# Ipsedo/MARLClassification

Hardware: AMD Instinct MI355X
Metric: agent-env-steps/sec (higher is better)
Workload: dtype f32; 1 GPU; RESISC45 256x256x3, 16 agents, 16 steps, f=12, README dims (configs[2]); full train iteration: rollout + A2C loss + BPTT backward + Adam; batch_per_gpu=256, global_batch=256, parallelism=dp1, rng=library (Philox4x32-10), launch=eager

## Files before the change

### marlclassification_amd/csrc/cnn.hip

```cpp
#include <stdlib.h>

#include <type_traits>

#include "common.h"

namespace marl {

template <bool FROM_OBS, typename PIX>
__global__ __launch_bounds__(256) void gather_im2col_kernel(
    const PIX* __restrict__ img, const int32_t* __restrict__ pos, float* __restrict__ cols,
    int ldk, int64_t rows, int nb, int c_img, int cin, int H, int W, int f, int rb) {
    extern __shared__ __attribute__((aligned(16))) float patch[];
    const int ff = f * f;
    const int pe = cin * ff;
    const int64_t row0 = (int64_t)blockIdx.x * rb;
    int nrow = (int)(rows - row0 < rb ? rows - row0 : rb);
    for (int idx = threadIdx.x; idx < nrow * pe; idx += 256) {
        const int lr = idx / pe, e = idx % pe;
        const int ci = e / ff, y = (e % ff) / f, x = e % f;
        const int64_t r = row0 + lr;
        float v;
        if (FROM_OBS) {
            v = (float)img[((r * c_img + ci) * f + y) * f + x];
        } else {
// ... 36 lines not shown
    const int rb = gather_rb(cin, f);
    const size_t lds = (size_t)rb * cin * f * f * sizeof(float);
    if (lds > 64 * 1024) {
        set_error("window %d too large for the gather kernel", f);
        return MARL_ELIMIT;
    }
    if (img_u8)
        hipLaunchKernelGGL((gather_im2col_kernel<false, unsigned char>),
                           dim3((unsigned)cdiv(rows, rb)), dim3(256), lds, st,
                           static_cast<const unsigned char*>(img), pos, cols, ldk, rows, nb, c_img,
                           cin, H, W, f, rb);
    else
        hipLaunchKernelGGL((gather_im2col_kernel<false, float>), dim3((unsigned)cdiv(rows, rb)),
                           dim3(256), lds, st, static_cast<const float*>(img), pos, cols, ldk, rows,
                           nb, c_img, cin, H, W, f, rb);
    MARL_LAUNCH_CHECK();
    return MARL_OK;
}

int launch_obs_im2col(const float* obs, float* cols, int ldk, int64_t rows, int c_img, int cin,
                      int f, hipStream_t st) {
    const int rb = gather_rb(cin, f);
    const size_t lds = (size_t)rb * cin * f * f * sizeof(float);
    if (lds > 64 * 1024) return MARL_ELIMIT;
    hipLaunchKernelGGL((gather_im2col_kernel<true, float>), dim3((unsigned)cdiv(rows, rb)), dim3(256),
                       lds, st, obs, (const int32_t*)nullptr, cols, ldk, rows, 1, c_img, cin, 0, 0,
                       f, rb);
    MARL_LAUNCH_CHECK();
    return MARL_OK;
}

#ifdef MARL_KERNEL_TS
int ts_begin(long long** dev, int call) {
    if (!*dev) (void)hipMalloc(dev, 16 * 48 * sizeof(long long));
    const char* e = getenv("MARL_TS_CALL");
    const int want = e ? atoi(e) : 100;
    if (call != want) return 0;
    (void)hipMemset(*dev, 0, 16 * 48 * sizeof(long long));
    return 1;
}
void ts_report(const char* tag, long long* dev, int waves) {
    static long long h[16 * 48];
    (void)hipMemcpy(h, dev, sizeof(h), hipMemcpyDeviceToHost);
    for (int w = 0; w < waves; w += (waves > 1 ? waves - 1 : 1)) {
        const long long* t = h + w * 48;
        fprintf(stderr, "[ts] %s wave %d/%d:", tag, w, waves);
        long long tot = 0;
        for (int i = 1; i < 48 && t[i]; ++i) {
            fprintf(stderr, " %lld", t[i] - t[i - 1]);
            tot += t[i] - t[i - 1];
        }
        fprintf(stderr, " | total %.2f us\n", tot / 100.0);
    }
}
#endif

typedef float cf32x4 __attribute__((ext_vector_type(4)));

__device__ __forceinline__ float cnn_silu(float y) { return silu_fast(y); }

__global__ __launch_bounds__(512) void cnn_fwd_kernel(const CnnFwdArgs A) {
    extern __shared__ __attribute__((aligned(16))) float lds[];
    float* patch = lds;
    float* gstat = lds + A.off_stat;
    __shared__ int64_t simg[16];
    __shared__ int spos[16][2];
    const int tid = threadIdx.x, lane = tid & 63, wave = tid >> 6;
    const int nthreads = blockDim.x, nwaves = nthreads >> 6;
    const int quad = lane >> 4, l16 = lane & 15;
    const int64_t row0 = (int64_t)blockIdx.x * A.rb;
    const int nrow = (int)(A.rows - row0 < A.rb ? A.rows - row0 : A.rb);

#ifdef MARL_KERNEL_TS
    MARL_TS_DECL(A.ts);
#endif
    MARL_TS();
    if (tid < nrow) {
        const int64_t r = row0 + tid;
        if (A.obs) {
            simg[tid] = r * A.c_img * A.f * A.f;
            spos[tid][0] = spos[tid][1] = 0;
        } else {
            simg[tid] = (r % A.nb) * A.c_img * (int64_t)A.H * A.W;
            spos[tid][0] = A.pos[r * 2];
            spos[tid][1] = A.pos[r * 2 + 1];
// ... 2876 lines not shown
```

### marlclassification_amd/csrc/common.h

```cpp
#pragma once

#include <hip/hip_runtime.h>
#include <stdint.h>
#include <stdio.h>

#include "../../include/marl_hip.h"
#include "split.h"

namespace marl {

constexpr int kWave = 64;

inline int p4(int x) { return (x + 3) & ~3; }
inline int64_t cdiv(int64_t a, int64_t b) { return (a + b - 1) / b; }

void set_error(const char* fmt, ...);

int tune_get(const char* key, int dflt);
int tune_set(const char* key, int value);

__device__ __forceinline__ float rcp_fast(float x) { return __builtin_amdgcn_rcpf(x); }
__device__ __forceinline__ float sigmoid_acc(float x) { return rcp_fast(1.0f + __expf(-x)); }
__device__ __forceinline__ float tanh_fast(float x) { return 1.0f - 2.0f * rcp_fast(1.0f + __expf(2.0f * x)); }
__device__ __forceinline__ float silu_fast(float y) { return y * sigmoid_acc(y); }
// ... 409 lines not shown

struct PanelLayer {
    const float* w;
    int ldw;
    const float* bias;
    const float* gamma;
    const float* beta;
    int n;
    float* z;
    int ldz;
    float* stats;
    float* a;
    int lda;
    char* a3;
    int a3_row0, a3_steps, a3_col0;
};
constexpr int kPanelMaxLayers = 4;
struct PanelFwdProb {
    const float* x;
    int ldx, k0;
    int agg_na, agg_nb;
    float* xbar;
    int m, nlayers;
    PanelLayer layer[kPanelMaxLayers];
    int by_batch, g_na, g_nb, agg_at, ld_xbar;
    const float* mix;
};
struct PanelFwdBatch {
    PanelFwdProb p[2];
    int count;
    int off_panel1, off_red, off_part, off_prm;
    int off_mix;
    int has_sample, panel_blocks;
    int ln_narrow_max;
    SampleArgs sample;
#ifdef MARL_KERNEL_TS
    long long* ts;
#endif
};
int panel_chain_supported(int na, int n_msg, int threads);
int panel_supported(int k0, int n0, int n1);
int launch_panel_fwd(PanelFwdBatch& b, hipStream_t st);

struct LstmBwdArgs {
    const float* dh;
    float* dc;
    float* gates;
    const float* c_prev;
    const float* c_new;
    int lddh, lddc, ldg, ldc, n;
    char* g3;
    int g3_row0, g3_steps;
    int skip_f32;
};
struct LstmBwdBatch {
    LstmBwdArgs a[2];
    int64_t rows;
    int vec4;
};
inline bool lstm_bwd_vec4_ok(const LstmBwdArgs& a) {
    return (a.n & 3) == 0 && (a.lddh & 3) == 0 && (a.lddc & 3) == 0 && (a.ldg & 3) == 0 && (a.ldc & 3) == 0;
}
__device__ __forceinline__ void lstm_cell_bwd_at(const LstmBwdArgs& A, int64_t r, int u, float dhv);
__device__ __forceinline__ void lstm_cell_bwd_elem(const LstmBwdArgs& A, int64_t rows, int64_t idx) {
    const int n = A.n;
    if (idx >= rows * n) return;
    const int64_t r = idx / n;
    const int u = (int)(idx % n);
    lstm_cell_bwd_at(A, r, u, A.dh[r * A.lddh + u]);
}
__device__ __forceinline__ void lstm_cell_bwd_at(const LstmBwdArgs& A, int64_t r, int u, float dhv) {
    const int n = A.n;
    float* g = A.gates + r * A.ldg + u;
    const float gi = g[0], gf = g[n], gg = g[2 * n], go = g[3 * n];
// ... 69 lines not shown
};
struct PanelBwdProb {
    const float* da;
    int ldda;
    const float* da2;
    int ldda2;
    int agg_na, agg_nb;
    int m, nlayers;
    PanelBwdLayer layer[kPanelMaxLayers];
    float* dx;
    int lddx, accumulate;
    int by_batch, g_na, g_nb, agg_at;
    int has_cellb;
    LstmBwdArgs cellb;
    int off_e, off_prm, off_colp, off_part, off_rowmap;
    const float* mix;
    int off_mix;
    int tail_lds;
    int has_cell, panel_blocks;
    LstmBwdArgs cell;
    int64_t cell_rows;
    int cell_vec4;
    int cellb_img_done, cell_img_done;
#ifdef MARL_KERNEL_TS
    long long* ts;
#endif
};
int panel_bwd_blocks(int m);
int panel_chain_blocks(int na, int nb);
int panel_chain_by_batch(int na);
int launch_panel_bwd(PanelBwdProb& p, hipStream_t st);

#ifdef MARL_KERNEL_TS
#define MARL_TS_DECL(ptr) long long* ts_ = (ptr); int tsi_ = 0
#define MARL_TS()                                                                         \
    if (ts_ && (threadIdx.x & 63) == 0 && blockIdx.x == 37 && blockIdx.y == 0 && tsi_ < 48) \
    ts_[(threadIdx.x >> 6) * 48 + tsi_++] = wall_clock64()
int ts_begin(long long** dev, int call);
void ts_report(const char* tag, long long* dev, int waves);
#else
#define MARL_TS_DECL(ptr)
#define MARL_TS()
#endif

struct FDiv {
    uint32_t d, m;
};
inline FDiv make_fdiv(int d) { return FDiv{(uint32_t)d, (uint32_t)(((1ull << 32) / (uint64_t)d) + 1)}; }
__device__ __forceinline__ int fdiv(int n, FDiv f) {
    return f.d == 1 ? n : (int)__umulhi((uint32_t)n, f.m);
}

struct CnnFwdLayer {
    const float *w, *bias, *gamma, *beta;
    float* cols;
    float* z;
    float* gst;
    int cin, cout, G, hin, hout, P, K, ldk;
    const float* wfrag;
};
struct CnnFwdArgs {
    const void* img;
    const float* obs;
    const int32_t* pos;
    int img_u8;
    int64_t rows;
    int nb, c_img, H, W, f, L;
    CnnFwdLayer layer[MARL_MAX_CNN_LAYERS];
    float* u;
    int ldu;
    char* u3;
    int u3_row0, u3_steps;
// ... 161 lines not shown
```

### marlclassification_amd/csrc/episode.hip

```cpp
#include <math.h>
#include <stdlib.h>
#include <string.h>

#include "common.h"

namespace marl {

struct Dims {
    int na, nb, ns;
    int64_t R, NR;
    int H, W, c_img, f;
    int L;
    int ch[MARL_MAX_CNN_LAYERS + 1];
    int grp[MARL_MAX_CNN_LAYERS];
    int hw[MARL_MAX_CNN_LAYERS + 1];
    int P[MARL_MAX_CNN_LAYERS];
    int K[MARL_MAX_CNN_LAYERS];
    int ldk[MARL_MAX_CNN_LAYERS];
    int nf, nin;
    int n_b, n_a, n_m, nm2, n_mo, n_d, nA, nC, nlb, nla;
    int ld_nin, ld_nb, ld_na, ld_nm, ld_nm2, ld_nmo, ld_nd, ld_nla, ld_nlb, ld_gb, ld_ga, ld_nC,
        ld_nA;
    int ld_dbl;
};
// ... 856 lines not shown
                                 c.at(c.e.ZE1, t), d.ld_nm2, R, d.nm2, c.wp(MARL_P_ENC_B0)),
                       gemm_prob(c.HCs(t + 1), d.ld_na, c.wp(MARL_P_POL_W0), d.ld_na, d.n_a,
                                 c.at(c.e.ZP1, t), d.ld_nla, R, d.nla, c.wp(MARL_P_POL_B0))));
    } else if (which == 1) {
        MARL_TRY(gemm1(c, gemm_prob(c.Hs(t + 1), d.ld_nb, c.wp(MARL_P_ENC_W0), d.ld_nb, d.n_b,
                                    c.at(c.e.ZE1, t), d.ld_nm2, R, d.nm2, c.wp(MARL_P_ENC_B0))));
    } else {
        MARL_TRY(gemm1(c, gemm_prob(c.HCs(t + 1), d.ld_na, c.wp(MARL_P_POL_W0), d.ld_na, d.n_a,
                                    c.at(c.e.ZP1, t), d.ld_nla, R, d.nla, c.wp(MARL_P_POL_B0))));
    }
    if (which & 2)
        MARL_TRY(launch_ln_silu_fwd(c.at(c.e.ZP1, t), d.ld_nla, c.wp(MARL_P_POL_LNW),
                                    c.wp(MARL_P_POL_LNB), c.at(c.e.AP1, t), d.ld_nla,
                                    c.at(c.e.STP1, t), d.R, d.nla, st));
    if (which & 1) {
        MARL_TRY(launch_ln_silu_fwd(c.at(c.e.ZE1, t), d.ld_nm2, c.wp(MARL_P_ENC_LN0W),
                                    c.wp(MARL_P_ENC_LN0B), c.at(c.e.AE1, t), d.ld_nm2,
                                    c.at(c.e.STE1, t), d.R, d.nm2, st));
        MARL_TRY(gemm1(c, gemm_prob(c.at(c.e.AE1, t), d.ld_nm2, c.wp(MARL_P_ENC_W1), d.ld_nm2,
                                    d.nm2, c.at(c.e.ZE2, t), d.ld_nm, R, d.n_m,
                                    c.wp(MARL_P_ENC_B1))));
        MARL_TRY(launch_ln_silu_fwd(c.at(c.e.ZE2, t), d.ld_nm, c.wp(MARL_P_ENC_LN1W),
                                    c.wp(MARL_P_ENC_LN1B), c.MSGs(t + 1), d.ld_nm,
                                    c.at(c.e.STE2, t), d.R, d.n_m, st));
    }
    return MARL_OK;
}

static bool use_chain(const Dims& d) {
    return use_panels(d) && panel_chain_supported(d.na, d.n_m, 256) && d.n_mo <= 384 && d.nm2 <= 384 &&
           d.n_m <= 384 && tune_get("panel_chain", 1) != 0 &&
           (!g_comm || d.n_b <= 384);
}
static int step_chain(const Ctx& c, int t) {
    const Dims& d = c.d;
    PanelFwdBatch pb{};
    pb.count = 2;
    PanelFwdProb& pe = pb.p[0];
    fill_enc_prob(c, t, pe);
    pe.by_batch = panel_chain_by_batch(d.na);
    pe.g_na = d.na;
    pe.g_nb = d.nb;
    if (t + 1 < d.ns) {
        fill_dec_layers(c, t + 1, pe.layer + 2);
        pe.nlayers = 4;
        pe.agg_at = 2;
        pe.xbar = c.at(c.e.MBAR, t + 1);
        pe.ld_xbar = d.ld_nm;
        pe.mix = g_comm;
    }
    fill_pol_prob(c, t, pb.p[1]);
    return launch_panel_fwd(pb, c.st);
}

static int step_core(const Ctx& c, int t, const StepIn& in) {
    MARL_TRY(step_cnn(c, t, in));
    MARL_TRY(step_decode(c, t));
    MARL_TRY(step_pos_lstm(c, t, in));
    return step_encode_policy(c, t, 3);
}

struct SideStream {
    hipStream_t s = nullptr;
    hipEvent_t ev[64];
    int next = 0;
    int init() {
        if (s) return MARL_OK;
        MARL_HIP_CHECK(hipStreamCreateWithFlags(&s, hipStreamNonBlocking));
        for (auto& e : ev) MARL_HIP_CHECK(hipEventCreateWithFlags(&e, hipEventDisableTiming));
        return MARL_OK;
    }
    int order(hipStream_t from, hipStream_t to) {
        hipEvent_t e = ev[next];
        next = (next + 1) % 64;
        MARL_HIP_CHECK(hipEventRecord(e, from));
        MARL_HIP_CHECK(hipStreamWaitEvent(to, e, 0));
        return MARL_OK;
    }
};
static SideStream g_side;

static bool use_side_stream() {
    static int enabled = -1;
    (void)enabled;
// ... 968 lines not shown
                               int train, void* stream) {
    Ctx c;
    SplitRegistryScope reg_scope;
    MARL_TRY(make_ctx(cfg, weights_ws, weights_ws_bytes, episode_ws, episode_ws_bytes, train, stream, c));
    if (!img || !pos0 || !h0 || !c0 || !hc0 || !cc0 || !step_preds || !step_logp || !step_values) {
        set_error("episode_forward: null argument");
        return MARL_EINVAL;
    }
    if (c.d.ns >= 65536) {
        set_error("episode_forward: more than 65535 steps");
        return MARL_ELIMIT;
    }
    const Dims& d = c.d;
    MARL_TRY(launch_i64_to_i32(pos0, c.POSs(0), d.R * 2, c.st));
    MARL_TRY(load_state(c, h0, c0, hc0, cc0, nullptr));
    StepIn in;
    in.img = img;
    in.img_u8 = cfg->img_u8 != 0;
    const bool side = use_side_stream();
    Ctx c2 = c;
    if (side) {
        MARL_TRY(g_side.init());
        c2.st = g_side.s;
    }
    bool decoded_ahead = false;
    const bool chain = !side && use_chain(d);
    for (int t = 0; t < d.ns; ++t) {
        MARL_TRY(step_cnn(c, t, in));
        if (side && t > 0)
            MARL_TRY(g_side.order(c2.st, c.st));
        else if (!decoded_ahead)
            MARL_TRY(step_decode(c, t));
        MARL_TRY(step_pos_lstm(c, t, in, t > 0));
        if (chain) {
            MARL_TRY(step_chain(c, t));
        } else if (side) {
            MARL_TRY(g_side.order(c.st, c2.st));
            MARL_TRY(step_encode_policy(c2, t, 1));
            if (t + 1 < d.ns) MARL_TRY(step_decode(c2, t + 1));
            MARL_TRY(step_encode_policy(c, t, 2));
        } else {
            MARL_TRY(step_encode_policy(c, t, 3));
        }
        SampleArgs a;
        fill_sample_args(c, cfg, t, a);
        a.noise = noise ? noise + (size_t)t * d.R * d.nA : nullptr;
        a.rng_on = !noise && !forced_actions;
        a.rng_seed = rng_seed ^ 0x9E3779B97F4A7C15ull;
        a.rng_ctr = (rng_offset << 16) + (uint64_t)t;
        a.rng_off_dev = counters ? &static_cast<const Counters*>(counters)->rng_offset : nullptr;
        a.forced = forced_actions ? forced_actions + (size_t)t * d.R : nullptr;
        a.step_pos = step_pos ? step_pos + (size_t)t * d.R * 2 : nullptr;
        a.step_actions = step_actions ? step_actions + (size_t)t * d.R : nullptr;
        a.step_logp = step_logp + (size_t)t * d.R;
        if (t + 1 < d.ns) {
            a.pe_W = c.wp(MARL_P_POS_W);
            a.pe_b = c.wp(MARL_P_POS_B);
            a.pe_gamma = c.wp(MARL_P_POS_LNW);
            a.pe_beta = c.wp(MARL_P_POS_LNB);
            a.pe_npos = c.at(c.e.NPOS, t + 1);
            a.pe_z = c.at(c.e.ZPOS, t + 1);
            a.pe_stats = c.at(c.e.STPOS, t + 1);
            a.pe_out = c.at(c.e.U, t + 1) + d.nf + d.n_mo;
            a.pe_ldz = d.ld_nd;
            a.pe_ldo = d.ld_nin;
            a.pe_nd = d.n_d;
            if (c.u3_by_producers) {
                a.pe_img = c.img(c.e.U3);
                a.pe_row0 = c.u3_row(t + 1);
                a.pe_steps = img_steps(d.nin);
                a.pe_col0 = d.nf + d.n_mo;
            }
        }
        decoded_ahead = chain && t + 1 < d.ns;
        if (!side && !chain && t + 1 < d.ns) MARL_TRY(step_decode(c, t + 1, &a, &decoded_ahead));
        if (chain || !decoded_ahead) MARL_TRY(launch_sample(a, c.st));
    }
    if (side) MARL_TRY(g_side.order(c2.st, c.st));
    MARL_TRY(heads_batched(c, 0, d.NR, step_values, step_preds));
    if (step_probs) MARL_TRY(launch_copy2d(c.PROBSs(0), d.nA, step_probs, d.nA, d.NR, d.nA, c.st));
    return MARL_OK;
}

int marl_episode_forward(const marl_config* cfg, const void* weights_ws, size_t weights_ws_bytes,
                         void* episode_ws, size_t episode_ws_bytes, const void* img, const int64_t* pos0, const float* h0, const float* c0,
                         const float* hc0, const float* cc0, const float* noise,
                         const int64_t* forced_actions, uint64_t rng_seed, uint64_t rng_offset,
                         const void* counters, float* step_preds, float* step_logp,
                         float* step_values, int64_t* step_pos, int64_t* step_actions, int train,
                         void* stream) {
    return episode_forward_all(cfg, weights_ws, weights_ws_bytes, episode_ws, episode_ws_bytes, img, pos0, h0, c0,
                               hc0, cc0, noise, forced_actions, rng_seed, rng_offset, counters, step_preds,
                               step_logp, step_values, step_pos, step_actions, nullptr, train, stream);
}

int marl_episode_forward_probs(const marl_config* cfg, const void* weights_ws, size_t weights_ws_bytes,
                               void* episode_ws, size_t episode_ws_bytes, const void* img, const int64_t* pos0,
                               const float* h0, const float* c0, const float* hc0, const float* cc0,
                               const float* noise, const int64_t* forced_actions, uint64_t rng_seed,
                               uint64_t rng_offset, const void* counters, float* step_preds, float* step_logp,
                               float* step_values, int64_t* step_pos, int64_t* step_actions, float* step_probs,
                               int train, void* stream) {
    if (!step_probs) {
        set_error("episode_forward_probs: null step_probs");
        return MARL_EINVAL;
    }
    return episode_forward_all(cfg, weights_ws, weights_ws_bytes, episode_ws, episode_ws_bytes, img, pos0, h0, c0,
                               hc0, cc0, noise, forced_actions, rng_seed, rng_offset, counters, step_preds,
                               step_logp, step_values, step_pos, step_actions, step_probs, train, stream);
// ... 567 lines not shown
    set_error("unknown debug buffer %s", name);
    return MARL_EINVAL;
}

int marl_plan_query(const marl_config* cfg, int train, const char* key, int* value) {
    Dims d;
    MARL_TRY(make_dims(cfg, d));
    (void)train;
    if (!key || !value) return MARL_EINVAL;
    if (!strcmp(key, "g3")) *value = g3_enabled(d);
    else if (!strcmp(key, "g3_model")) *value = g3_model_ok(d);
    else if (!strcmp(key, "g3_lstm")) *value = g3_enabled(d) && tune_get("g3_lstm", 1) != 0;
    else if (!strcmp(key, "g3_tn")) *value = g3_enabled(d) && g3_tn_enabled(d);
    else if (!strcmp(key, "lstm_plan") || !strcmp(key, "small_r")) {
        int plan = 0;
        if (g3_enabled(d) && tune_get("g3_lstm", 1) != 0) {
            G3Batch b{};
            b.count = 2;
            b.p[0].m = b.p[1].m = (int)d.R;
            b.p[0].n = d.n_b;
            b.p[1].n = d.n_a;
            plan = tune_get("g3_lstm_variant", 0);
            if (!plan) plan = g3_lstm_plan(b);
        }
        *value = !strcmp(key, "small_r") ? (plan == 3 || plan == 4) : plan;
    }
    else if (!strcmp(key, "g3_tn_cell"))
        *value = g3_enabled(d) && g3_tn_enabled(d) && g3_tn_cell_ok(4 * d.n_b, d.nin, d.n_b, d.NR) &&
                 g3_tn_cell_ok(4 * d.n_a, d.nin, d.n_a, d.NR);
    else if (!strcmp(key, "g3_tn_pipe")) *value = tune_get("g3_tn_pipe", 1) != 0;
    else if (!strcmp(key, "wgrad3")) *value = tune_get("wgrad3", 1) != 0;
    else if (!strcmp(key, "comm")) *value = g_comm != nullptr;
    else if (!strcmp(key, "panel_chain")) *value = use_chain(d) && !use_side_stream();
    else if (!strcmp(key, "comm_form"))
        *value = g_comm ? ((use_chain(d) && !use_side_stream()) ? 5 : use_panels(d) ? 3 : 4)
                        : (use_chain(d) && !use_side_stream()) ? 0 : use_panels(d) ? 1 : 2;
    else {
        set_error("unknown plan key %s", key);
        return MARL_EINVAL;
    }
    return MARL_OK;
}

}
namespace marl {
__global__ void normalize_positions_kernel(const int64_t* __restrict__ pos, float* __restrict__ out,
                                           int rows, int H, int W) {
    const int r = blockIdx.x * blockDim.x + threadIdx.x;
    if (r >= rows) return;
    out[r * 2] = (float)pos[r * 2] / (float)H;
    out[r * 2 + 1] = (float)pos[r * 2 + 1] / (float)W;
}
}
extern "C" {

int marl_normalize_positions(const int64_t* pos, float* out, int rows, int h, int w, void* stream) {
    if (!pos || !out || rows < 1 || h < 1 || w < 1) {
        set_error("normalize_positions: bad argument");
        return MARL_EINVAL;
    }
    hipLaunchKernelGGL(normalize_positions_kernel, dim3((unsigned)cdiv(rows, 256)), dim3(256), 0,
                       static_cast<hipStream_t>(stream), pos, out, rows, h, w);
    MARL_LAUNCH_CHECK();
    return MARL_OK;
}

// ... 119 lines not shown
```

### marlclassification_amd/csrc/panel.hip

```cpp
#include <stdlib.h>

#include "common.h"
#include "sample.h"

namespace marl {

typedef float f32x4 __attribute__((ext_vector_type(4)));

__device__ __forceinline__ void lds_barrier() {
    asm volatile("s_waitcnt lgkmcnt(0)\n\ts_barrier" ::: "memory");
}
__device__ __forceinline__ float silu_p(float y) { return silu_fast(y); }
__device__ __forceinline__ float silu_grad_p(float y) { return silu_grad_fast(y); }

constexpr int kPanelRows = 16;
constexpr int kPanelMaxWaves = 12;
constexpr int kPanelMaxCols = 6;

__host__ __device__ inline int panel_stride(int k) { return ((k + 15) & ~15) + 4; }

__device__ __forceinline__ void panel_gemm(f32x4 (&acc)[2], const float* in, int stride, int K,
                                           const float* __restrict__ w, int ldw, int n, int j,
                                           int kbeg, int kend, int lane) {
    const int K4 = (K + 3) & ~3;
// ... 100 lines not shown
#pragma unroll
            for (int u = 0; u < NC; ++u) {
                const int c = lane + 64 * u;
                const float d = c < n ? v[u] - mean : 0.f;
                v[u] = d;
                q += d * d;
            }
            const float rstd = 1.0f / sqrtf(wave_sum(q) * inv_n + 1e-5f);
            float* arow = Lr.a + (size_t)(row < 0 ? 0 : row) * Lr.lda;
#pragma unroll
            for (int u = 0; u < NC; ++u) {
                const int c = lane + 64 * u;
                if (c < n) {
                    const float av = silu_p(v[u] * rstd * g[u] + bt[u]);
                    zr[c] = av;
                    if (row >= 0) arow[c] = av;
                }
            }
            if (Lr.stats && lane == 0 && row >= 0) {
                Lr.stats[(size_t)row * 2] = mean;
                Lr.stats[(size_t)row * 2 + 1] = rstd;
            }
            if (Lr.a3 && row >= 0) {
                for (int c4 = 4 * lane; c4 < n; c4 += 256) {
                    const float4 t = *reinterpret_cast<const float4*>(zr + c4);
                    const int col = Lr.a3_col0 + c4;
                    img_store4(Lr.a3 + img_off((int64_t)Lr.a3_row0 + row, col >> 4, Lr.a3_steps), col, t.x, t.y, t.z, t.w);
                }
            }
        }
    }
}

template <int SAMPLE, bool MIX = false>
__global__ __launch_bounds__(768, 6) void panel_fwd_kernel(const PanelFwdBatch B) {
    extern __shared__ __attribute__((aligned(16))) float lds[];
    if (SAMPLE > 0 && (int)blockIdx.x >= B.panel_blocks) {
        const int r = ((int)blockIdx.x - B.panel_blocks) * (int)(blockDim.x >> 6) + (int)(threadIdx.x >> 6);
        if (r >= B.sample.R) return;
        constexpr int MAXA = SAMPLE > 0 ? SAMPLE : 4;
        float p[MAXA];
        SamplePre<MAXA> S;
        sample_prefetch<MAXA, false>(B.sample, r, threadIdx.x & 63, S);
        sample_row_logits<MAXA>(B.sample, r, p, threadIdx.x & 63);
        sample_finish<MAXA>(B.sample, r, p, threadIdx.x & 63, S);
        return;
    }
    const PanelFwdProb& P = B.p[blockIdx.y];
    const int m0 = blockIdx.x * kPanelRows;
    const int bpb = P.by_batch;
    if (bpb ? (int)blockIdx.x * bpb >= P.g_nb : m0 >= P.m) return;
    const int tid = threadIdx.x, lane = tid & 63, wave = tid >> 6, nwaves = blockDim.x >> 6;
    int* rowmap = reinterpret_cast<int*>(lds + B.off_red);
    if (tid < kPanelRows) {
        int r = m0 + tid < P.m ? m0 + tid : -1;
        if (bpb) {
            const int a = tid / bpb, b = (int)blockIdx.x * bpb + (tid - a * bpb);
            r = (a < P.g_na && b < P.g_nb) ? a * P.g_nb + b : -1;
        }
        rowmap[tid] = r;
    }
    lds_barrier();
    const int quad = lane >> 4, l16 = lane & 15;
#ifdef MARL_KERNEL_TS
    MARL_TS_DECL(B.ts);
#endif
    MARL_TS();
    float* X = lds;
    float* Y = lds + B.off_panel1;
    float* part = lds + B.off_part;
// ... 177 lines not shown
        f32x4 acc[2];
        if (active) panel_gemm(acc, in, stride, K, Lr.w, Lr.ldw, n, j, kbeg, kend, lane);
        MARL_TS();
        panel_ksum(acc, part, nt, ks, j, s, lane, active);
        MARL_TS();

        const int ys = panel_stride(n), n16 = (n + 15) & ~15;
        if (active && s == 0) {
#pragma unroll
            for (int t = 0; t < 2; ++t) {
                const int col = j * 32 + 16 * t + l16;
                const bool cv = col < n;
                const float bv = cv ? lbias[col] : 0.f;
#pragma unroll
                for (int r = 0; r < 4; ++r) {
                    const int lr = 4 * quad + r;
                    const float zv = cv ? acc[t][r] + bv : 0.f;
                    if (col < n16) outp[lr * ys + col] = zv;
                }
            }
        }
        MARL_TS();
        lds_barrier();
        MARL_TS();
        if (n <= B.ln_narrow_max)
            panel_ln_rows<2>(Lr, outp, ys, n, lgamma, lbeta, rowmap, wave, nwaves, lane);
        else
            panel_ln_rows<kPanelMaxCols>(Lr, outp, ys, n, lgamma, lbeta, rowmap, wave, nwaves, lane);
        MARL_TS();
        lds_barrier();
        MARL_TS();
        K = n;
    }
}

constexpr size_t kPanelMaxLds = 144 * 1024;

static int panel_waves_for(int k, int n) {
    const int nt = (n + 31) / 32;
    const int want = (((k + 15) & ~15) + 63) / 64;
    int w = nt * want;
    if (w < nt) w = nt;
    return w > kPanelMaxWaves ? (nt > kPanelMaxWaves ? -1 : (kPanelMaxWaves / nt) * nt) : w;
}

int panel_chain_supported(int na, int n_msg, int threads) {
    const int K16 = (n_msg + 15) & ~15;
    return na >= 1 && na <= kPanelRows && kPanelRows * (K16 / 4) <= 2 * threads;
}

int panel_supported(int k0, int n0, int n1) {
    if (n0 > 32 * kPanelMaxWaves || n1 > 32 * kPanelMaxWaves) return 0;
    if (n0 > 64 * kPanelMaxCols || n1 > 64 * kPanelMaxCols) return 0;
    const int kx = k0 > n1 ? k0 : n1;
    const size_t lds = (size_t)(kPanelRows * panel_stride(kx) + kPanelRows * panel_stride(n0) +
                                (kPanelMaxWaves + 1) * 32 + (kPanelMaxWaves - 1) * 512 +
                                3 * (n0 + n1) + 16) * 4;
    return lds <= kPanelMaxLds;
}

int launch_panel_fwd(PanelFwdBatch& b, hipStream_t st) {
    int waves = 1, x0 = 0, x1 = 0;
    for (int i = 0; i < b.count; ++i) {
        const PanelFwdProb& p = b.p[i];
        for (int l = 0; l < p.nlayers; ++l) {
            const int w = panel_waves_for(l == 0 ? p.k0 : p.layer[l - 1].n, p.layer[l].n);
            if (w < 0) {
                set_error("panel kernel: layer width %d too large", p.layer[l].n);
                return MARL_ELIMIT;
            }
            waves = w > waves ? w : waves;
        }
        int s0 = kPanelRows * panel_stride(p.k0), s1 = 0;
        for (int l = 0; l < p.nlayers; ++l) {
            const int v = kPanelRows * panel_stride(p.layer[l].n);
            if (l & 1)
                s0 = v > s0 ? v : s0;
            else
                s1 = v > s1 ? v : s1;
        }
        if (p.agg_at > 0 && (p.by_batch < 1 || p.g_na * p.by_batch > kPanelRows || p.agg_at >= p.nlayers ||
                             !panel_chain_supported(p.g_na, p.layer[p.agg_at - 1].n, 256))) {
            set_error("panel kernel: in-panel message mean outside its range");
            return MARL_ELIMIT;
        }
        if (p.mix && (p.agg_at <= 0 || i != 0 || (b.has_sample && b.count == 1))) {
            set_error("panel kernel: a mixing matrix needs the in-panel aggregation of problem 0");
            return MARL_ELIMIT;
        }
        x0 = s0 > x0 ? s0 : x0;
        x1 = s1 > x1 ? s1 : x1;
    }
    const bool mixed = b.count > 0 && b.p[0].mix != nullptr;
    if (waves < 4) waves = 4;
    b.off_panel1 = x0;
    b.off_red = x0 + x1;
    b.off_part = b.off_red + (kPanelMaxWaves + 1) * 32;
    b.off_prm = b.off_part + (waves - 1) * 512;
    int prm = 0;
    for (int i = 0; i < b.count; ++i) {
        int q = 0;
        for (int l = 0; l < b.p[i].nlayers; ++l) q += 3 * b.p[i].layer[l].n;
        prm = q > prm ? q : prm;
    }
    b.off_mix = b.off_prm + prm + 16;
    const size_t lds = (size_t)(b.off_mix + (mixed ? kPanelRows * kPanelRows : 0)) * sizeof(float);
    if (lds > kPanelMaxLds) {
        set_error("panel kernel: shape outside its range");
        return MARL_ELIMIT;
    }
    static bool raised = false;
    if (!raised) {
        const void* kerns[4] = {reinterpret_cast<const void*>(panel_fwd_kernel<0>),
                                reinterpret_cast<const void*>(panel_fwd_kernel<4>),
                                reinterpret_cast<const void*>(panel_fwd_kernel<MARL_MAX_ACTIONS>),
                                reinterpret_cast<const void*>(panel_fwd_kernel<0, true>)};
        for (const void* kf : kerns)
            MARL_HIP_CHECK(hipFuncSetAttribute(kf, hipFuncAttributeMaxDynamicSharedMemorySize, (int)kPanelMaxLds));
        raised = true;
    }
    b.ln_narrow_max = 128;
    unsigned pblocks = 0;
    for (int i = 0; i < b.count; ++i) {
        const PanelFwdProb& p = b.p[i];
        const unsigned nblk = p.by_batch > 0 ? (unsigned)cdiv(p.g_nb, p.by_batch) : (unsigned)cdiv(p.m, kPanelRows);
        pblocks = nblk > pblocks ? nblk : pblocks;
    }
#ifdef MARL_KERNEL_TS
    static long long* d_ts = nullptr;
    static int calls = 0;
    const int rec = ts_begin(&d_ts, calls++);
    b.ts = rec ? d_ts : nullptr;
#endif
    prof_before(4, st);
    if (b.has_sample && b.count == 1) {
        b.panel_blocks = (int)pblocks;
        const unsigned sblocks = (unsigned)cdiv(b.sample.R, waves);
        if (b.sample.nA <= 4)
            hipLaunchKernelGGL(panel_fwd_kernel<4>, dim3(pblocks + sblocks, 1), dim3(64 * waves), lds, st, b);
        else
            hipLaunchKernelGGL(panel_fwd_kernel<MARL_MAX_ACTIONS>, dim3(pblocks + sblocks, 1), dim3(64 * waves), lds, st, b);
    } else {
        b.has_sample = 0;
        if (mixed)
            hipLaunchKernelGGL((panel_fwd_kernel<0, true>), dim3(pblocks, (unsigned)b.count), dim3(64 * waves),
                               lds, st, b);
        else
            hipLaunchKernelGGL(panel_fwd_kernel<0>, dim3(pblocks, (unsigned)b.count), dim3(64 * waves), lds, st, b);
    }
    prof_after(4, st);
    MARL_LAUNCH_CHECK();
#ifdef MARL_KERNEL_TS
    if (rec) {
        fprintf(stderr, "[ts] panel_fwd count %d sample %d waves %d lds %zu\n", b.count, b.has_sample, waves, lds);
        ts_report("panel_fwd", d_ts, waves);
    }
#endif
    return MARL_OK;
}

constexpr int kBwdMaxCols = kPanelMaxCols;

template <bool CELL, int MAXC, bool MIX = false>
__global__ __launch_bounds__(768, 4) void panel_bwd_kernel(const PanelBwdProb P) {
    extern __shared__ __attribute__((aligned(16))) float lds[];
    if (CELL && (int)blockIdx.x >= P.panel_blocks) {
        const int64_t idx = (int64_t)((int)blockIdx.x - P.panel_blocks) * blockDim.x + threadIdx.x;
        if (P.cell_vec4)
            lstm_cell_bwd_elem4(P.cell, P.cell_rows, idx);
        else
            lstm_cell_bwd_elem(P.cell, P.cell_rows, idx);
        return;
    }
    const int m0 = blockIdx.x * kPanelRows;
    const int bpb = P.by_batch;
    if (bpb ? (int)blockIdx.x * bpb >= P.g_nb : m0 >= P.m) return;
    const int tid = threadIdx.x, lane = tid & 63, wave = tid >> 6, nwaves = blockDim.x >> 6;
    const int quad = lane >> 4, l16 = lane & 15;
    float* D = lds;
    float* E = lds + P.off_e;
    float* prm = lds + P.off_prm;
    float* colp = lds + P.off_colp;
    float* part = lds + P.off_part;
    int* rowmap = reinterpret_cast<int*>(lds + P.off_rowmap);
    if (tid < kPanelRows) {
        int r = m0 + tid < P.m ? m0 + tid : -1;
        if (bpb) {
            const int a = tid / bpb, b = (int)blockIdx.x * bpb + (tid - a * bpb);
// ... 487 lines not shown
```

### marlclassification_amd/csrc/sample.h

```cpp
#pragma once

#include "common.h"

namespace marl {

__device__ __forceinline__ float sample_silu(float y) { return silu_fast(y); }

struct Philox4 {
    uint32_t x, y, z, w;
};
__device__ __forceinline__ Philox4 philox4x32_10(uint64_t key, uint64_t ctr_hi, uint32_t c0, uint32_t c1) {
    uint32_t k0 = (uint32_t)key, k1 = (uint32_t)(key >> 32);
    Philox4 c{c0, c1, (uint32_t)ctr_hi, (uint32_t)(ctr_hi >> 32)};
#pragma unroll
    for (int i = 0; i < 10; ++i) {
        const uint32_t hi0 = __umulhi(0xD2511F53u, c.x), lo0 = 0xD2511F53u * c.x;
        const uint32_t hi1 = __umulhi(0xCD9E8D57u, c.z), lo1 = 0xCD9E8D57u * c.z;
        c = Philox4{hi1 ^ c.y ^ k0, lo1, hi0 ^ c.w ^ k1, lo0};
        k0 += 0x9E3779B9u;
        k1 += 0xBB67AE85u;
    }
    return c;
}
__device__ __forceinline__ float philox_u01(uint32_t v) { return ((float)(v >> 8) + 0.5f) * (1.0f / 16777216.0f); }

template <int MAXA>
__device__ __forceinline__ void sample_logits_chunk(const SampleArgs& A, const float (&a)[8], int base,
                                                    float (&p)[MAXA], int lane) {
#pragma unroll
    for (int j0 = 0; j0 < MAXA; j0 += 4) {
        if (j0 < A.nA) {
            float wv[4][8];
#pragma unroll
            for (int jj = 0; jj < 4; ++jj) {
                const int j = j0 + jj < A.nA ? j0 + jj : A.nA - 1;
                const float* wj = A.w1 + (size_t)j * A.ldw;
#pragma unroll
                for (int u = 0; u < 8; ++u) {
                    const int k = base + lane + 64 * u;
                    const float v = wj[k < A.nla ? k : 0];
                    wv[jj][u] = k < A.nla ? v : 0.f;
                }
            }
#pragma unroll
            for (int jj = 0; jj < 4; ++jj) {
                float s = 0.f;
#pragma unroll
                for (int u = 0; u < 8; ++u) s += a[u] * wv[jj][u];
                p[j0 + jj] += s;
            }
        }
    }
}

template <int MAXA>
__device__ __forceinline__ void sample_row_logits(const SampleArgs& A, int r, float (&p)[MAXA], int lane) {
    const float* ar = A.a_pol + (size_t)r * A.ld_a;
#pragma unroll
    for (int j = 0; j < MAXA; ++j) p[j] = 0.f;
    for (int base = 0; base < A.nla; base += 512) {
        float a[8];
#pragma unroll
        for (int u = 0; u < 8; ++u) {
            const int k = base + lane + 64 * u;
            const float v = ar[k < A.nla ? k : 0];
            a[u] = k < A.nla ? v : 0.f;
        }
        sample_logits_chunk<MAXA>(A, a, base, p, lane);
    }
}

template <int MAXA>
struct SamplePre {
    float b1[MAXA];
    float nz[MAXA];
    uint64_t ctr;
    int pi0, pi1, forced;
    bool pe_fast;
    float4 qb, qw[4], qg, qbt;
};
__device__ __forceinline__ bool sample_pe_fast(const SampleArgs& A) {
    const uintptr_t al = (uintptr_t)A.pe_W | (uintptr_t)A.pe_b | (uintptr_t)A.pe_gamma | (uintptr_t)A.pe_beta |
                         (uintptr_t)A.pe_z | (uintptr_t)A.pe_out;
    return A.pe_W && A.step_logp && (al & 15) == 0 && A.pe_nd <= 256 && ((A.pe_nd | A.pe_ldz | A.pe_ldo) & 3) == 0 &&
           (A.pe_col0 & 3) == 0;
}
template <int MAXA, bool PE = true>
__device__ __forceinline__ void sample_prefetch(const SampleArgs& A, int r, int lane, SamplePre<MAXA>& S) {
#pragma unroll
    for (int j = 0; j < MAXA; ++j) S.b1[j] = A.b1[j < A.nA ? j : A.nA - 1];
    if (A.noise) {
        const float* nr = A.noise + (size_t)r * A.nA;
#pragma unroll
        for (int j = 0; j < MAXA; ++j) S.nz[j] = nr[j < A.nA ? j : A.nA - 1];
    } else {
#pragma unroll
        for (int j = 0; j < MAXA; ++j) S.nz[j] = 1.0f;
    }
    S.ctr = A.rng_ctr + (A.rng_off_dev ? (*A.rng_off_dev << 16) : 0ull);
    S.pi0 = S.pi1 = S.forced = 0;
    if (A.step_logp) {
        S.pi0 = A.pos_in[r * 2];
        S.pi1 = A.pos_in[r * 2 + 1];
        if (A.forced) S.forced = (int)A.forced[r];
    }
    S.pe_fast = PE && sample_pe_fast(A);
    if (PE && S.pe_fast) {
        const int j4 = 4 * lane < A.pe_nd ? 4 * lane : 0;
        S.qb = *reinterpret_cast<const float4*>(A.pe_b + j4);
        S.qg = *reinterpret_cast<const float4*>(A.pe_gamma + j4);
        S.qbt = *reinterpret_cast<const float4*>(A.pe_beta + j4);
#pragma unroll
        for (int q = 0; q < 4; ++q) S.qw[q] = *reinterpret_cast<const float4*>(A.pe_W + 4 * (j4 + q));
    }
}

template <int MAXA>
__device__ __forceinline__ void sample_finish(const SampleArgs& A, int r, float (&p)[MAXA], int lane,
                                              const SamplePre<MAXA>& S) {
    float mx = -INFINITY;
#pragma unroll
    for (int j = 0; j < MAXA; ++j) {
        if (j < A.nA) {
            p[j] = wave_sum(p[j]) + S.b1[j];
            mx = fmaxf(mx, p[j]);
        } else {
            p[j] = 0.f;
        }
    }
    float den = 0.f;
#pragma unroll
    for (int j = 0; j < MAXA; ++j)
        if (j < A.nA) {
            p[j] = expf(p[j] - mx);
            den += p[j];
        }
    int act = 0;
    float best = -INFINITY, pa = 0.f;
#pragma unroll
    for (int j = 0; j < MAXA; ++j)
        if (j < A.nA) {
            p[j] = p[j] / den;
            if (A.noise) {
                const float sc = p[j] / S.nz[j];
                if (sc > best) {
                    best = sc;
                    act = j;
// ... 140 lines not shown
```

Measured before the change: 8.963 million agent-env-steps/s.

## Fuse action sampling into the panel forward kernel as an epilogue

```diff
diff --git a/marlclassification_amd/csrc/cnn.hip b/marlclassification_amd/csrc/cnn.hip
--- a/marlclassification_amd/csrc/cnn.hip
+++ b/marlclassification_amd/csrc/cnn.hip
@@ -92,25 +92,28 @@
 
 #ifdef MARL_KERNEL_TS
 int ts_begin(long long** dev, int call) {
-    if (!*dev) (void)hipMalloc(dev, 16 * 48 * sizeof(long long));
+    constexpr size_t bytes = (size_t)kTsRoles * kTsWaves * kTsSlots * sizeof(long long);
+    if (!*dev) (void)hipMalloc(dev, bytes);
     const char* e = getenv("MARL_TS_CALL");
     const int want = e ? atoi(e) : 100;
     if (call != want) return 0;
-    (void)hipMemset(*dev, 0, 16 * 48 * sizeof(long long));
+    (void)hipMemset(*dev, 0, bytes);
     return 1;
 }
-void ts_report(const char* tag, long long* dev, int waves) {
-    static long long h[16 * 48];
+void ts_report(const char* tag, long long* dev, int waves, int role) {
+    static long long h[kTsRoles * kTsWaves * kTsSlots];
     (void)hipMemcpy(h, dev, sizeof(h), hipMemcpyDeviceToHost);
+    const long long t00 = h[0];
     for (int w = 0; w < waves; w += (waves > 1 ? waves - 1 : 1)) {
-        const long long* t = h + w * 48;
+        const long long* t = h + (role * kTsWaves + w) * kTsSlots;
         fprintf(stderr, "[ts] %s wave %d/%d:", tag, w, waves);
         long long tot = 0;
-        for (int i = 1; i < 48 && t[i]; ++i) {
+        for (int i = 1; i < kTsSlots && t[i]; ++i) {
             fprintf(stderr, " %lld", t[i] - t[i - 1]);
             tot += t[i] - t[i - 1];
         }
-        fprintf(stderr, " | total %.2f us\n", tot / 100.0);
+        fprintf(stderr, " | total %.2f us, start %+.2f end %+.2f us\n", tot / 100.0, (t[0] - t00) / 100.0,
+                (t[0] + tot - t00) / 100.0);
     }
 }
 #endif
diff --git a/marlclassification_amd/csrc/common.h b/marlclassification_amd/csrc/common.h
--- a/marlclassification_amd/csrc/common.h
+++ b/marlclassification_amd/csrc/common.h
@@ -465,6 +465,7 @@
     int off_panel1, off_red, off_part, off_prm;
     int off_mix;
     int has_sample, panel_blocks;
+    int epi_prob;
     int ln_narrow_max;
     SampleArgs sample;
 #ifdef MARL_KERNEL_TS
@@ -473,6 +474,7 @@
 };
 int panel_chain_supported(int na, int n_msg, int threads);
 int panel_supported(int k0, int n0, int n1);
+int panel_sample_supported(int n_actions);
 int launch_panel_fwd(PanelFwdBatch& b, hipStream_t st);
 
 struct LstmBwdArgs {
@@ -608,12 +610,13 @@
 int launch_panel_bwd(PanelBwdProb& p, hipStream_t st);
 
 #ifdef MARL_KERNEL_TS
+constexpr int kTsWaves = 16, kTsSlots = 48, kTsRoles = 2;
 #define MARL_TS_DECL(ptr) long long* ts_ = (ptr); int tsi_ = 0
-#define MARL_TS()                                                                         \
-    if (ts_ && (threadIdx.x & 63) == 0 && blockIdx.x == 37 && blockIdx.y == 0 && tsi_ < 48) \
-    ts_[(threadIdx.x >> 6) * 48 + tsi_++] = wall_clock64()
+#define MARL_TS()                                                                              \
+    if (ts_ && (threadIdx.x & 63) == 0 && blockIdx.x == 37 && blockIdx.y < kTsRoles && tsi_ < kTsSlots) \
+    ts_[((int)blockIdx.y * kTsWaves + (threadIdx.x >> 6)) * kTsSlots + tsi_++] = wall_clock64()
 int ts_begin(long long** dev, int call);
-void ts_report(const char* tag, long long* dev, int waves);
+void ts_report(const char* tag, long long* dev, int waves, int role = 0);
 #else
 #define MARL_TS_DECL(ptr)
 #define MARL_TS()
diff --git a/marlclassification_amd/csrc/episode.hip b/marlclassification_amd/csrc/episode.hip
--- a/marlclassification_amd/csrc/episode.hip
+++ b/marlclassification_amd/csrc/episode.hip
@@ -912,7 +912,15 @@
            d.n_m <= 384 && tune_get("panel_chain", 1) != 0 &&
            (!g_comm || d.n_b <= 384);
 }
-static int step_chain(const Ctx& c, int t) {
+static bool use_panel_sample(const Dims& d) {
+    static int enabled = -1;
+    if (enabled < 0) {
+        const char* e = getenv("MARL_PANEL_SAMPLE");
+        enabled = (e && e[0] == '0') ? 0 : 1;
+    }
+    return enabled && panel_sample_supported(d.nA);
+}
+static int step_chain(const Ctx& c, int t, const SampleArgs* sample = nullptr) {
     const Dims& d = c.d;
     PanelFwdBatch pb{};
     pb.count = 2;
@@ -930,6 +938,10 @@
         pe.mix = g_comm;
     }
     fill_pol_prob(c, t, pb.p[1]);
+    if (sample && use_panel_sample(d)) {
+        pb.epi_prob = 2;
+        pb.sample = *sample;
+    }
     return launch_panel_fwd(pb, c.st);
 }
 
@@ -1964,16 +1976,6 @@
         else if (!decoded_ahead)
             MARL_TRY(step_decode(c, t));
         MARL_TRY(step_pos_lstm(c, t, in, t > 0));
-        if (chain) {
-            MARL_TRY(step_chain(c, t));
-        } else if (side) {
-            MARL_TRY(g_side.order(c.st, c2.st));
-            MARL_TRY(step_encode_policy(c2, t, 1));
-            if (t + 1 < d.ns) MARL_TRY(step_decode(c2, t + 1));
-            MARL_TRY(step_encode_policy(c, t, 2));
-        } else {
-            MARL_TRY(step_encode_policy(c, t, 3));
-        }
         SampleArgs a;
         fill_sample_args(c, cfg, t, a);
         a.noise = noise ? noise + (size_t)t * d.R * d.nA : nullptr;
@@ -2004,9 +2006,19 @@
                 a.pe_col0 = d.nf + d.n_mo;
             }
         }
+        if (chain) {
+            MARL_TRY(step_chain(c, t, &a));
+        } else if (side) {
+            MARL_TRY(g_side.order(c.st, c2.st));
+            MARL_TRY(step_encode_policy(c2, t, 1));
+            if (t + 1 < d.ns) MARL_TRY(step_decode(c2, t + 1));
+            MARL_TRY(step_encode_policy(c, t, 2));
+        } else {
+            MARL_TRY(step_encode_policy(c, t, 3));
+        }
         decoded_ahead = chain && t + 1 < d.ns;
         if (!side && !chain && t + 1 < d.ns) MARL_TRY(step_decode(c, t + 1, &a, &decoded_ahead));
-        if (chain || !decoded_ahead) MARL_TRY(launch_sample(a, c.st));
+        if (chain ? !use_panel_sample(d) : !decoded_ahead) MARL_TRY(launch_sample(a, c.st));
     }
     if (side) MARL_TRY(g_side.order(c2.st, c.st));
     MARL_TRY(heads_batched(c, 0, d.NR, step_values, step_preds));
@@ -2640,6 +2652,7 @@
     else if (!strcmp(key, "wgrad3")) *value = tune_get("wgrad3", 1) != 0;
     else if (!strcmp(key, "comm")) *value = g_comm != nullptr;
     else if (!strcmp(key, "panel_chain")) *value = use_chain(d) && !use_side_stream();
+    else if (!strcmp(key, "panel_sample")) *value = use_chain(d) && !use_side_stream() && use_panel_sample(d);
     else if (!strcmp(key, "comm_form"))
         *value = g_comm ? ((use_chain(d) && !use_side_stream()) ? 5 : use_panels(d) ? 3 : 4)
                         : (use_chain(d) && !use_side_stream()) ? 0 : use_panels(d) ? 1 : 2;
diff --git a/marlclassification_amd/csrc/panel.hip b/marlclassification_amd/csrc/panel.hip
--- a/marlclassification_amd/csrc/panel.hip
+++ b/marlclassification_amd/csrc/panel.hip
@@ -156,10 +156,43 @@
     }
 }
 
-template <int SAMPLE, bool MIX = false>
+template <int MAXA, bool UNI>
+__device__ __forceinline__ void panel_sample_rows(const SampleArgs& A0, const float* outp, int ys, const int* rowmap,
+                                                  int wave, int nwaves, int lane) {
+    for (int lr = __builtin_amdgcn_readfirstlane(wave); lr < kPanelRows; lr += nwaves) {
+        const int row = __builtin_amdgcn_readfirstlane(rowmap[lr]);
+        if (row < 0) continue;
+        int ln = (int)__builtin_amdgcn_mbcnt_hi(~0u, __builtin_amdgcn_mbcnt_lo(~0u, 0u));
+        asm volatile("" : "+v"(ln));
+        int zero = 0;
+        asm volatile("" : "+s"(zero));
+        const SampleArgs& A = (&A0)[zero];
+        float p[MAXA];
+        SamplePre<MAXA> S;
+        sample_prefetch_row<MAXA>(A, row, ln, S);
+        sample_row_logits_at<MAXA, kPanelMaxCols>(A, outp + lr * ys, p, ln);
+        if (UNI) {
+            auto uni = [](float v) { return __int_as_float(__builtin_amdgcn_readfirstlane(__float_as_int(v))); };
+#pragma unroll
+            for (int j = 0; j < MAXA; ++j) {
+                S.b1[j] = uni(S.b1[j]);
+                S.nz[j] = uni(S.nz[j]);
+            }
+            S.ctr = ((uint64_t)(uint32_t)__builtin_amdgcn_readfirstlane((int)(S.ctr >> 32)) << 32) |
+                    (uint32_t)__builtin_amdgcn_readfirstlane((int)S.ctr);
+            S.pi0 = __builtin_amdgcn_readfirstlane(S.pi0);
+            S.pi1 = __builtin_amdgcn_readfirstlane(S.pi1);
+            S.forced = __builtin_amdgcn_readfirstlane(S.forced);
+        }
+        sample_prefetch_pe<MAXA>(A, ln, S);
+        sample_finish<MAXA>(A, row, p, ln, S);
+    }
+}
+
+template <int SAMPLE, bool MIX = false, bool EPI = false>
 __global__ __launch_bounds__(768, 6) void panel_fwd_kernel(const PanelFwdBatch B) {
     extern __shared__ __attribute__((aligned(16))) float lds[];
-    if (SAMPLE > 0 && (int)blockIdx.x >= B.panel_blocks) {
+    if (!EPI && SAMPLE > 0 && (int)blockIdx.x >= B.panel_blocks) {
         const int r = ((int)blockIdx.x - B.panel_blocks) * (int)(blockDim.x >> 6) + (int)(threadIdx.x >> 6);
         if (r >= B.sample.R) return;
         constexpr int MAXA = SAMPLE > 0 ? SAMPLE : 4;
@@ -403,6 +436,11 @@
         MARL_TS();
         K = n;
     }
+    if (EPI && (int)(&P - B.p) + 1 == B.epi_prob) {
+        constexpr int MAXA = SAMPLE > 0 ? SAMPLE : 4;
+        panel_sample_rows<MAXA, MIX>(B.sample, (P.nlayers & 1) ? Y : X, panel_stride(K), rowmap, wave, nwaves, lane);
+        MARL_TS();
+    }
 }
 
 constexpr size_t kPanelMaxLds = 144 * 1024;
@@ -419,6 +457,8 @@
     const int K16 = (n_msg + 15) & ~15;
     return na >= 1 && na <= kPanelRows && kPanelRows * (K16 / 4) <= 2 * threads;
 }
+
+int panel_sample_supported(int n_actions) { return n_actions >= 1 && n_actions <= 4; }
 
 int panel_supported(int k0, int n0, int n1) {
     if (n0 > 32 * kPanelMaxWaves || n1 > 32 * kPanelMaxWaves) return 0;
@@ -482,10 +522,12 @@
     }
     static bool raised = false;
     if (!raised) {
-        const void* kerns[4] = {reinterpret_cast<const void*>(panel_fwd_kernel<0>),
+        const void* kerns[6] = {reinterpret_cast<const void*>(panel_fwd_kernel<0>),
                                 reinterpret_cast<const void*>(panel_fwd_kernel<4>),
                                 reinterpret_cast<const void*>(panel_fwd_kernel<MARL_MAX_ACTIONS>),
-                                reinterpret_cast<const void*>(panel_fwd_kernel<0, true>)};
+                                reinterpret_cast<const void*>(panel_fwd_kernel<0, true>),
+                                reinterpret_cast<const void*>(panel_fwd_kernel<4, false, true>),
+                                reinterpret_cast<const void*>(panel_fwd_kernel<4, true, true>)};
         for (const void* kf : kerns)
             MARL_HIP_CHECK(hipFuncSetAttribute(kf, hipFuncAttributeMaxDynamicSharedMemorySize, (int)kPanelMaxLds));
         raised = true;
@@ -503,8 +545,24 @@
     const int rec = ts_begin(&d_ts, calls++);
     b.ts = rec ? d_ts : nullptr;
 #endif
+    if (b.epi_prob) {
+        const PanelFwdProb* p = b.epi_prob >= 1 && b.epi_prob <= b.count ? &b.p[b.epi_prob - 1] : nullptr;
+        if (!p || !panel_sample_supported(b.sample.nA) || p->nlayers < 1 || p->m != b.sample.R ||
+            p->layer[p->nlayers - 1].a != b.sample.a_pol || p->layer[p->nlayers - 1].n != b.sample.nla) {
+            set_error("panel kernel: the sampling epilogue needs the problem whose last layer writes its activations");
+            return MARL_EINVAL;
+        }
+    }
     prof_before(4, st);
-    if (b.has_sample && b.count == 1) {
+    if (b.epi_prob) {
+        b.has_sample = 0;
+        if (mixed)
+            hipLaunchKernelGGL((panel_fwd_kernel<4, true, true>), dim3(pblocks, (unsigned)b.count), dim3(64 * waves),
+                               lds, st, b);
+        else
+            hipLaunchKernelGGL((panel_fwd_kernel<4, false, true>), dim3(pblocks, (unsigned)b.count), dim3(64 * waves),
+                               lds, st, b);
+    } else if (b.has_sample && b.count == 1) {
         b.panel_blocks = (int)pblocks;
         const unsigned sblocks = (unsigned)cdiv(b.sample.R, waves);
         if (b.sample.nA <= 4)
@@ -523,8 +581,10 @@
     MARL_LAUNCH_CHECK();
 #ifdef MARL_KERNEL_TS
     if (rec) {
-        fprintf(stderr, "[ts] panel_fwd count %d sample %d waves %d lds %zu\n", b.count, b.has_sample, waves, lds);
+        fprintf(stderr, "[ts] panel_fwd count %d sample %d epilogue %d waves %d lds %zu\n", b.count, b.has_sample,
+                b.epi_prob, waves, lds);
         ts_report("panel_fwd", d_ts, waves);
+        if (b.count == 2) ts_report("panel_fwd role 1", d_ts, waves, 1);
     }
 #endif
     return MARL_OK;
diff --git a/marlclassification_amd/csrc/sample.h b/marlclassification_amd/csrc/sample.h
--- a/marlclassification_amd/csrc/sample.h
+++ b/marlclassification_amd/csrc/sample.h
@@ -24,19 +24,19 @@
 }
 __device__ __forceinline__ float philox_u01(uint32_t v) { return ((float)(v >> 8) + 0.5f) * (1.0f / 16777216.0f); }
 
-template <int MAXA>
-__device__ __forceinline__ void sample_logits_chunk(const SampleArgs& A, const float (&a)[8], int base,
+template <int MAXA, int NU = 8>
+__device__ __forceinline__ void sample_logits_chunk(const SampleArgs& A, const float (&a)[NU], int base,
                                                     float (&p)[MAXA], int lane) {
 #pragma unroll
     for (int j0 = 0; j0 < MAXA; j0 += 4) {
         if (j0 < A.nA) {
-            float wv[4][8];
+            float wv[4][NU];
 #pragma unroll
             for (int jj = 0; jj < 4; ++jj) {
                 const int j = j0 + jj < A.nA ? j0 + jj : A.nA - 1;
                 const float* wj = A.w1 + (size_t)j * A.ldw;
 #pragma unroll
-                for (int u = 0; u < 8; ++u) {
+                for (int u = 0; u < NU; ++u) {
                     const int k = base + lane + 64 * u;
                     const float v = wj[k < A.nla ? k : 0];
                     wv[jj][u] = k < A.nla ? v : 0.f;
@@ -46,28 +46,31 @@
             for (int jj = 0; jj < 4; ++jj) {
                 float s = 0.f;
 #pragma unroll
-                for (int u = 0; u < 8; ++u) s += a[u] * wv[jj][u];
+                for (int u = 0; u < NU; ++u) s += a[u] * wv[jj][u];
                 p[j0 + jj] += s;
             }
         }
     }
 }
 
-template <int MAXA>
-__device__ __forceinline__ void sample_row_logits(const SampleArgs& A, int r, float (&p)[MAXA], int lane) {
-    const float* ar = A.a_pol + (size_t)r * A.ld_a;
+template <int MAXA, int NU = 8>
+__device__ __forceinline__ void sample_row_logits_at(const SampleArgs& A, const float* ar, float (&p)[MAXA], int lane) {
 #pragma unroll
     for (int j = 0; j < MAXA; ++j) p[j] = 0.f;
-    for (int base = 0; base < A.nla; base += 512) {
-        float a[8];
-#pragma unroll
-        for (int u = 0; u < 8; ++u) {
+    for (int base = 0; base < (NU < 8 ? 1 : A.nla); base += 512) {
+        float a[NU];
+#pragma unroll
+        for (int u = 0; u < NU; ++u) {
             const int k = base + lane + 64 * u;
             const float v = ar[k < A.nla ? k : 0];
             a[u] = k < A.nla ? v : 0.f;
         }
-        sample_logits_chunk<MAXA>(A, a, base, p, lane);
-    }
+        sample_logits_chunk<MAXA, NU>(A, a, base, p, lane);
+    }
+}
+template <int MAXA>
+__device__ __forceinline__ void sample_row_logits(const SampleArgs& A, int r, float (&p)[MAXA], int lane) {
+    sample_row_logits_at<MAXA>(A, A.a_pol + (size_t)r * A.ld_a, p, lane);
 }
 
 template <int MAXA>
@@ -85,8 +88,8 @@
     return A.pe_W && A.step_logp && (al & 15) == 0 && A.pe_nd <= 256 && ((A.pe_nd | A.pe_ldz | A.pe_ldo) & 3) == 0 &&
            (A.pe_col0 & 3) == 0;
 }
-template <int MAXA, bool PE = true>
-__device__ __forceinline__ void sample_prefetch(const SampleArgs& A, int r, int lane, SamplePre<MAXA>& S) {
+template <int MAXA>
+__device__ __forceinline__ void sample_prefetch_row(const SampleArgs& A, int r, int lane, SamplePre<MAXA>& S) {
 #pragma unroll
     for (int j = 0; j < MAXA; ++j) S.b1[j] = A.b1[j < A.nA ? j : A.nA - 1];
     if (A.noise) {
@@ -104,8 +107,12 @@
         S.pi1 = A.pos_in[r * 2 + 1];
         if (A.forced) S.forced = (int)A.forced[r];
     }
-    S.pe_fast = PE && sample_pe_fast(A);
-    if (PE && S.pe_fast) {
+    S.pe_fast = false;
+}
+template <int MAXA>
+__device__ __forceinline__ void sample_prefetch_pe(const SampleArgs& A, int lane, SamplePre<MAXA>& S) {
+    S.pe_fast = sample_pe_fast(A);
+    if (S.pe_fast) {
         const int j4 = 4 * lane < A.pe_nd ? 4 * lane : 0;
         S.qb = *reinterpret_cast<const float4*>(A.pe_b + j4);
         S.qg = *reinterpret_cast<const float4*>(A.pe_gamma + j4);
@@ -113,6 +120,11 @@
 #pragma unroll
         for (int q = 0; q < 4; ++q) S.qw[q] = *reinterpret_cast<const float4*>(A.pe_W + 4 * (j4 + q));
     }
+}
+template <int MAXA, bool PE = true>
+__device__ __forceinline__ void sample_prefetch(const SampleArgs& A, int r, int lane, SamplePre<MAXA>& S) {
+    sample_prefetch_row<MAXA>(A, r, lane, S);
+    if (PE) sample_prefetch_pe<MAXA>(A, lane, S);
 }
 
 template <int MAXA>
```

Measured after the change: 9.082 million agent-env-steps/s (median of 6 runs). +1.3%, better.
